# ModuRL/ModuRL_Gym

Measured on NVIDIA B200. Metric: env-steps/sec (CartPole-v1, 2^24 envs), higher is better.
Workload: dtype f32

## Files before the change

### modurl_gym_b200/csrc/mgym_api.cu

```cuda
#include <dlfcn.h>

#include <cmath>
#include <cstdarg>
#include <cstdio>
#include <cstdlib>
#include <cstring>
#include <limits>
#include <mutex>
#include <new>
#include <string>

#include "../../include/mgym.h"
#include "mgym_kernels.cuh"

#if defined(__has_include)
#if __has_include(<nccl.h>)
#include <nccl.h>
#define MGYM_HAVE_NCCL_H 1
#endif
#endif
namespace {
#ifdef MGYM_HAVE_NCCL_H
constexpr int kNcclFloat64 = (int)ncclFloat64, kNcclSum = (int)ncclSum;
static_assert(kNcclFloat64 == 8 && kNcclSum == 0, "NCCL enum values changed: update the header-less fallback below");
#else
constexpr int kNcclFloat64 = 8, kNcclSum = 0;
#endif
}

using namespace mgym;

struct mgym_env {
  int kind = 0;
  uint64_t n = 0;
  int device = 0;
  uint64_t seed = 0;
  mgym_config cfg{};
  int cnt_mode = CNT_U32;
  bool vec4 = false;

  float* state = nullptr;
  void* steps = nullptr;
  uint32_t* sbt = nullptr;
  float* ep_return = nullptr;
  float* reset_pool = nullptr;
  uint64_t pool_len = 0;
  unsigned long long* stats = nullptr;
  uint32_t* bad_action = nullptr;
  float* params = nullptr;
  bool redraw = false;
  float redraw_lo[MAX_PARAMS] = {}, redraw_hi[MAX_PARAMS] = {};

  uint64_t t = 0;
  uint64_t n_resets = 0;
  EnvConsts k{};
  int num_sms = 0;

  void* h_actions = nullptr;
  float* h_obs = nullptr;
  float* h_reward = nullptr;
  uint8_t* h_flags = nullptr;
  unsigned long long* work = nullptr;
  uint64_t work_issued[3] = {0, 0, 0};
  int work_slot = 0;
  unsigned long long* clock = nullptr;
  uint64_t call_tickets = 0;
  cudaStream_t pipe_stream[2] = {nullptr, nullptr};
  cudaEvent_t pipe_event[3] = {nullptr, nullptr, nullptr};
};

namespace {

thread_local std::string g_last_error;

int fail(int code, const char* fmt, ...) {
  char buf[512];
  va_list ap;
  va_start(ap, fmt);
  vsnprintf(buf, sizeof(buf), fmt, ap);
  va_end(ap);
  g_last_error = buf;
  return code;
}

#define MGYM_CUDA(expr)                                                                            \
  do {                                                                                             \
    cudaError_t e_ = (expr);                                                                       \
    if (e_ != cudaSuccess)                                                                         \
      return fail(e_ == cudaErrorMemoryAllocation ? MGYM_ERR_OUT_OF_MEMORY : MGYM_ERR_CUDA,        \
                  "%s failed: %s (%s:%d)", #expr, cudaGetErrorString(e_), __FILE__, __LINE__);    \
  } while (0)

struct DeviceGuard {
  int prev = -1;
  bool switched = false;
  explicit DeviceGuard(int dev) {
    if (cudaGetDevice(&prev) == cudaSuccess && prev != dev) switched = cudaSetDevice(dev) == cudaSuccess;
  }
  ~DeviceGuard() {
    if (switched) cudaSetDevice(prev);
  }
};

constexpr int kStateDim[MGYM_NUM_KINDS] = {4, 2, 2, 2, 4};
constexpr int kObsDim[MGYM_NUM_KINDS] = {4, 2, 2, 3, 6};
constexpr int kContinuous[MGYM_NUM_KINDS] = {0, 0, 1, 1, 0};
constexpr int kNumActions[MGYM_NUM_KINDS] = {2, 3, 0, 0, 3};
const char* const kNames[MGYM_NUM_KINDS] = {"CartPole-v1", "MountainCar-v0", "MountainCarContinuous-v0",
                                            "Pendulum-v1", "Acrobot-v1"};

constexpr int kNumParams[MGYM_NUM_KINDS] = {6, 2, 2, 3, 0};
const char* const kParamNames[MGYM_NUM_KINDS][6] = {
    {"gravity", "masscart", "masspole", "length", "force_mag", "tau"},
    {"force", "gravity"},
    {"power", "gravity"},
    {"g", "m", "l"},
    {}};
// ... 74 lines not shown
  p.n = e->n;
  p.first = 0;
  p.ld = e->n;
  p.seed = e->seed;
  p.keys = philox_keys(e->seed);
  p.t_dev = e->cfg.device_clock ? e->clock : nullptr;
  p.base_dev = nullptr;
  p.env_base = e->cfg.env_index_base;
  p.t = e->t;
  p.k = e->k;
  return p;
}

constexpr int kMaxDevices = 64;

struct OccupancyCache {
  static constexpr int kSlots = 256;
  std::mutex mu;
  const void* key[kSlots] = {};
  int dev[kSlots] = {};
  int per_sm[kSlots] = {};
  int used = 0;
  int find(const void* k, int d) {
    std::lock_guard<std::mutex> lock(mu);
    for (int i = 0; i < used; ++i)
      if (key[i] == k && dev[i] == d) return per_sm[i];
    return 0;
  }
  void put(const void* k, int d, int v) {
    std::lock_guard<std::mutex> lock(mu);
    if (used < kSlots) key[used] = k, dev[used] = d, per_sm[used] = v, ++used;
  }
};
OccupancyCache g_occupancy;

template <typename KP>
int launch_persistent(void (*kernel)(KP), const mgym_env* e, const KP& p, uint64_t groups, cudaStream_t st) {
  constexpr int threads = 256;
  int per_sm = g_occupancy.find(reinterpret_cast<const void*>(kernel), e->device);
  if (per_sm == 0) {
    MGYM_CUDA(cudaOccupancyMaxActiveBlocksPerMultiprocessor(&per_sm, kernel, threads, 0));
    if (per_sm < 1) per_sm = 1;
    g_occupancy.put(reinterpret_cast<const void*>(kernel), e->device, per_sm);
  }
  uint64_t blocks = (uint64_t)e->num_sms * per_sm;
  const uint64_t need = (groups + threads - 1) / threads;
  if (blocks > need) blocks = need;
  if (blocks < 1) blocks = 1;
  kernel<<<(unsigned)blocks, threads, 0, st>>>(p);
  MGYM_CUDA(cudaGetLastError());
  return MGYM_OK;
}

template <int KIND, int CNT, bool AUTO = true, bool PARAMS = false, bool REDRAW = false>
int launch_step_tma(const mgym_env* ce, const KParams<PARAMS, REDRAW>& p_in, cudaStream_t st) {
  mgym_env* e = const_cast<mgym_env*>(ce);
  KParams<PARAMS, REDRAW> p = p_in;
  using L = TmaLayout<KIND, CNT, AUTO, PARAMS>;
  auto kernel = step_kernel_tma<KIND, CNT, AUTO, PARAMS, REDRAW>;
  constexpr int threads = TMA_THREADS;
  static int cached_per_sm[kMaxDevices] = {};
  int per_sm = e->device < kMaxDevices ? cached_per_sm[e->device] : 0;
  if (per_sm == 0) {
    MGYM_CUDA(cudaFuncSetAttribute(kernel, cudaFuncAttributeMaxDynamicSharedMemorySize, (int)L::SMEM_BYTES));
    MGYM_CUDA(cudaOccupancyMaxActiveBlocksPerMultiprocessor(&per_sm, kernel, threads, L::SMEM_BYTES));
    if (per_sm < 1) per_sm = 1;
    if (e->device < kMaxDevices) cached_per_sm[e->device] = per_sm;
  }
  const uint64_t slots = (uint64_t)e->num_sms * per_sm;
  const uint64_t tiles = p.n / TMA_TILE;
  uint64_t blocks = tiles < slots ? tiles : slots;
  if (blocks < 1) blocks = 1;
  p.work_counter = e->work + e->work_slot;
  if (p.t_dev && e->work_slot == 0) {
    p.base_dev = e->clock + 1;
    if (p.adv_clock)
      p.adv_tickets = tiles + blocks;
    else
      e->call_tickets += tiles + blocks;
  } else {
    p.work_base = e->work_issued[e->work_slot];
    e->work_issued[e->work_slot] += tiles + blocks;
  }
  cudaLaunchConfig_t cfg{};
  cfg.gridDim = dim3((unsigned)blocks);
  cfg.blockDim = dim3(threads);
  cfg.dynamicSmemBytes = L::SMEM_BYTES;
  cfg.stream = st;
  cudaLaunchAttribute attr[1];
  attr[0].id = cudaLaunchAttributeProgrammaticStreamSerialization;
  attr[0].val.programmaticStreamSerializationAllowed = 1;
  cfg.attrs = attr;
  cfg.numAttrs = 1;
  MGYM_CUDA(cudaLaunchKernelEx(&cfg, kernel, p));
  return MGYM_OK;
}

template <int KIND, int V, bool ROLLOUT, bool PARAMS = false, bool REDRAW = false, bool FINAL = false>
int dispatch_mode(const mgym_env* e, const KParams<PARAMS, REDRAW>& p, cudaStream_t st) {
  static_assert(!FINAL || ROLLOUT, "final observations are a rollout form");
  const uint64_t groups = p.n / V;
  const bool autor = e->cfg.auto_reset != 0;
  if constexpr (!ROLLOUT && V == 4) {
    if constexpr (!REDRAW) {
      if (!autor && p.n % TMA_TILE == 0) return launch_step_tma<KIND, CNT_U32, false, PARAMS>(e, p, st);
    }
    if (autor && p.n % TMA_TILE == 0) {
      if constexpr (KIND == 0) {
        return launch_step_tma<KIND, CNT_S16, true, PARAMS, REDRAW>(e, p, st);
      } else {
        switch (e->cnt_mode) {
          case CNT_S16: return launch_step_tma<KIND, CNT_S16, true, PARAMS, REDRAW>(e, p, st);
          case CNT_S32_LAZY: return launch_step_tma<KIND, CNT_S32_LAZY, true, PARAMS, REDRAW>(e, p, st);
          default: return launch_step_tma<KIND, CNT_S32, true, PARAMS, REDRAW>(e, p, st);
        }
      }
    }
    if (p.n > TMA_TILE) {
      KParams<PARAMS, REDRAW> head = p, tail = p;
      head.adv_dt = 0;
      head.n = p.n - p.n % TMA_TILE;
      tail.first = p.first + head.n;
      tail.n = p.n - head.n;
      int rc = dispatch_mode<KIND, 4, false, PARAMS, REDRAW>(e, head, st);
      if (rc != MGYM_OK) return rc;
      return dispatch_mode<KIND, 4, false, PARAMS, REDRAW>(e, tail, st);
    }
  }
  [[maybe_unused]] const bool full = ROLLOUT && V == 4 && autor && p.n % (32 * V) == 0 && p.obs_out && p.reward_out &&
                                     p.flags_out;
#define MGYM_LAUNCH(AUTO_, CNT_)                                                                         \
  do {                                                                                                   \
    if constexpr (ROLLOUT) {                                                                             \
      if constexpr (AUTO_ && V == 4) {                                                                   \
        if (full)                                                                                        \
// ... 197 lines not shown
}

int mgym_space_action(int kind, float* low, float* high) {
  if (!valid_kind(kind) || !low || !high) return fail(MGYM_ERR_BAD_ARGUMENT, "mgym_space_action: bad argument");
  if (kind == MGYM_MOUNTAIN_CAR_CONTINUOUS_V0) {
    *low = -1.0f, *high = 1.0f;
  } else if (kind == MGYM_PENDULUM_V1) {
    *low = -2.0f, *high = 2.0f;
  } else {
    *low = 0.0f, *high = (float)(kNumActions[kind] - 1);
  }
  return MGYM_OK;
}

int mgym_config_default(int kind, mgym_config* cfg) {
  if (!valid_kind(kind) || !cfg) return fail(MGYM_ERR_BAD_ARGUMENT, "mgym_config_default: bad argument");
  memset(cfg, 0, sizeof(*cfg));
  cfg->struct_size = sizeof(mgym_config);
  cfg->auto_reset = 1;
  cfg->sutton_barto_reward = 0;
  cfg->is_euler = 1;
  cfg->goal_velocity = 0.0f;
  cfg->track_stats = 1;
  cfg->validate_actions = 0;
  cfg->env_index_base = 0;
  cfg->device_clock = 0;
  cfg->track_returns = 0;
  switch (kind) {
    case MGYM_MOUNTAIN_CAR_CONTINUOUS_V0: cfg->max_episode_steps = 999; break;
    case MGYM_PENDULUM_V1: cfg->max_episode_steps = 200; break;
    case MGYM_ACROBOT_V1: cfg->max_episode_steps = 500; break;
    default: cfg->max_episode_steps = 0;
  }
  return MGYM_OK;
}

int mgym_destroy(mgym_env* e) {
  if (!e) return MGYM_OK;
  DeviceGuard guard(e->device);
  cudaFree(e->clock);
  cudaFree(e->state);
  cudaFree(e->steps);
  cudaFree(e->sbt);
  cudaFree(e->ep_return);
  cudaFree(e->reset_pool);
  cudaFree(e->stats);
  cudaFree(e->bad_action);
  cudaFree(e->params);
  cudaFree(e->h_actions);
  cudaFree(e->h_obs);
  cudaFree(e->h_reward);
  cudaFree(e->h_flags);
  cudaFree(e->work);
  for (auto& s : e->pipe_stream)
    if (s) cudaStreamDestroy(s);
  for (auto& ev : e->pipe_event)
    if (ev) cudaEventDestroy(ev);
  delete e;
  return MGYM_OK;
}

int mgym_create(int kind, uint64_t num_envs, int device_ordinal, uint64_t seed, const mgym_config* cfg_in,
                mgym_env** out) {
  if (!out) return fail(MGYM_ERR_BAD_ARGUMENT, "mgym_create: out is NULL");
  *out = nullptr;
  if (!valid_kind(kind)) return fail(MGYM_ERR_BAD_ARGUMENT, "mgym_create: unknown kind %d", kind);
  if (num_envs == 0) return fail(MGYM_ERR_BAD_ARGUMENT, "mgym_create: num_envs must be > 0");
  mgym_config cfg;
  mgym_config_default(kind, &cfg);
  if (cfg_in) {
    if (cfg_in->struct_size != sizeof(mgym_config))
      return fail(MGYM_ERR_BAD_ARGUMENT, "mgym_create: cfg->struct_size %u != %zu", cfg_in->struct_size,
                  sizeof(mgym_config));
    cfg = *cfg_in;
  }
  if (cfg.max_episode_steps < 0) return fail(MGYM_ERR_BAD_ARGUMENT, "mgym_create: max_episode_steps < 0");

  int n_dev = 0;
  cudaError_t ce = cudaGetDeviceCount(&n_dev);
  if (ce != cudaSuccess || n_dev == 0)
    return fail(MGYM_ERR_CUDA, "mgym_create: no CUDA device (%s); there is no CPU fallback",
                ce == cudaSuccess ? "device count is 0" : cudaGetErrorString(ce));
  if (device_ordinal < 0 || device_ordinal >= n_dev)
    return fail(MGYM_ERR_BAD_ARGUMENT, "mgym_create: device %d out of range [0,%d)", device_ordinal, n_dev);

  mgym_env* e = new (std::nothrow) mgym_env();
  if (!e) return fail(MGYM_ERR_OUT_OF_MEMORY, "mgym_create: host allocation failed");
  e->kind = kind;
  e->n = num_envs;
  e->device = device_ordinal;
  e->seed = seed;
  e->cfg = cfg;
  e->k = make_consts(kind, cfg);
  e->vec4 = (num_envs % 4 == 0) && (cfg.env_index_base % 4 == 0);

  if (!cfg.auto_reset) {
    e->cnt_mode = CNT_U32;
  } else if (kind == MGYM_CARTPOLE_V1) {
    e->cnt_mode = CNT_S16;
  } else if (cfg.max_episode_steps > 0 && cfg.max_episode_steps <= 65535) {
    e->cnt_mode = CNT_S16;
  } else if (cfg.max_episode_steps > 65535) {
    e->cnt_mode = CNT_S32;
  } else {
    e->cnt_mode = CNT_S32_LAZY;
  }

  DeviceGuard guard(device_ordinal);
  int rc = [&]() -> int {
    cudaDeviceProp prop;
    MGYM_CUDA(cudaGetDeviceProperties(&prop, device_ordinal));
    e->num_sms = prop.multiProcessorCount;
    const size_t n = (size_t)num_envs;
    MGYM_CUDA(cudaMalloc(&e->state, sizeof(float) * kStateDim[kind] * n));
    MGYM_CUDA(cudaMemset(e->state, 0, sizeof(float) * kStateDim[kind] * n));
    MGYM_CUDA(cudaMalloc(&e->steps, counter_width(e->cnt_mode) * n));
    MGYM_CUDA(cudaMemset(e->steps, 0, counter_width(e->cnt_mode) * n));
    if (!cfg.auto_reset && kind == MGYM_CARTPOLE_V1) {
      MGYM_CUDA(cudaMalloc(&e->sbt, sizeof(uint32_t) * n));
      fill_u32_kernel<<<(unsigned)((n + 255) / 256), 256>>>(e->sbt, 1u, n);
      MGYM_CUDA(cudaGetLastError());
    }
    const bool analytic = kind == MGYM_CARTPOLE_V1 || kind == MGYM_MOUNTAIN_CAR_V0 || kind == MGYM_ACROBOT_V1;
    if (cfg.auto_reset && cfg.track_stats && cfg.track_returns && !analytic) {
      MGYM_CUDA(cudaMalloc(&e->ep_return, sizeof(float) * n));
      MGYM_CUDA(cudaMemset(e->ep_return, 0, sizeof(float) * n));
    }
    MGYM_CUDA(cudaMalloc(&e->stats, 5 * sizeof(unsigned long long)));
    MGYM_CUDA(cudaMemset(e->stats, 0, 5 * sizeof(unsigned long long)));
    MGYM_CUDA(cudaMalloc(&e->clock, 3 * sizeof(unsigned long long)));
    MGYM_CUDA(cudaMemset(e->clock, 0, 3 * sizeof(unsigned long long)));
    MGYM_CUDA(cudaMalloc(&e->work, 4 * sizeof(unsigned long long)));
    MGYM_CUDA(cudaMemset(e->work, 0, 4 * sizeof(unsigned long long)));
    MGYM_CUDA(cudaMalloc(&e->bad_action, sizeof(uint32_t)));
    MGYM_CUDA(cudaMemset(e->bad_action, 0, sizeof(uint32_t)));
    MGYM_CUDA(cudaDeviceSynchronize());
    return MGYM_OK;
  }();
  if (rc != MGYM_OK) {
    std::string keep = g_last_error;
    mgym_destroy(e);
    g_last_error = keep;
    return rc;
  }
  *out = e;
  return MGYM_OK;
}

uint64_t mgym_num_envs(const mgym_env* e) { return e ? e->n : 0; }
int mgym_kind_of(const mgym_env* e) { return e ? e->kind : MGYM_ERR_BAD_ARGUMENT; }
uint64_t mgym_step_index(const mgym_env* ce) {
  if (!ce) return 0;
  mgym_env* e = const_cast<mgym_env*>(ce);
  if (e->cfg.device_clock) {
    DeviceGuard guard(e->device);
    unsigned long long t = e->t;
    if (cudaDeviceSynchronize() == cudaSuccess &&
        cudaMemcpy(&t, e->clock, sizeof(t), cudaMemcpyDeviceToHost) == cudaSuccess)
      e->t = t;
    else
      cudaGetLastError();
  }
  return e->t;
}
float* mgym_state_ptr(mgym_env* e) { return e ? e->state : nullptr; }

int mgym_reset_masked(mgym_env* e, const uint8_t* mask, float* obs_out, void* stream) {
  if (e) {
    if (int rc = refuse_capture(e, (cudaStream_t)stream, "mgym_reset", false)) return rc;
  }
  if (!e) return fail(MGYM_ERR_BAD_ARGUMENT, "mgym_reset: env is NULL");
  DeviceGuard guard(e->device);
  cudaStream_t st = (cudaStream_t)stream;
  KernelParams p = base_params(e);
  p.obs_out = obs_out;
  int rc;
  switch (e->kind) {
    case 0: rc = launch_reset_kind<0>(e, p, mask, st); break;
    case 1: rc = launch_reset_kind<1>(e, p, mask, st); break;
    case 2: rc = launch_reset_kind<2>(e, p, mask, st); break;
    case 3: rc = launch_reset_kind<3>(e, p, mask, st); break;
    default: rc = launch_reset_kind<4>(e, p, mask, st); break;
  }
  if (rc == MGYM_OK && e->redraw) {
    reset_redraw_params_kernel<<<(unsigned)((e->n + 255) / 256), 256, 0, st>>>(
        e->params, e->n, kNumParams[e->kind], mask, e->seed, e->cfg.env_index_base, e->n_resets, redraw_box(e));
// ... 217 lines not shown
                (unsigned long long)h.pool_len, (unsigned long long)mine.pool_len);
  const bool with_params = (h.has_params & 1u) != 0 && kNumParams[e->kind] > 0;
  const bool with_ranges = with_params && (h.has_params & 2u) != 0;
  if (blob_bytes < checkpoint_bytes(e, with_params, with_ranges))
    return fail(MGYM_ERR_BAD_ARGUMENT, "mgym_checkpoint_load: truncated blob");
  float lo[MAX_PARAMS] = {}, hi[MAX_PARAMS] = {};
  if (with_ranges) {
    const size_t np = (size_t)kNumParams[e->kind];
    const uint8_t* r = static_cast<const uint8_t*>(blob) + checkpoint_bytes(e, true, false);
    memcpy(lo, r, sizeof(float) * np);
    memcpy(hi, r + sizeof(float) * np, sizeof(float) * np);
    if (int rc = check_redraw_ranges(e->kind, lo, hi, "mgym_checkpoint_load")) return rc;
  }
  DeviceGuard guard(e->device);
  if (with_params && !e->params) MGYM_CUDA(cudaMalloc(&e->params, param_bytes(e)));
  cudaStream_t st = (cudaStream_t)stream;
  const size_t n = (size_t)e->n;
  const uint8_t* in = static_cast<const uint8_t*>(blob) + sizeof(h);
  auto push = [&](void* dev, size_t bytes) -> int {
    if (bytes) MGYM_CUDA(cudaMemcpyAsync(dev, in, bytes, cudaMemcpyHostToDevice, st));
    in += bytes;
    return MGYM_OK;
  };
  int rc;
  if ((rc = push(e->state, sizeof(float) * kStateDim[e->kind] * n))) return rc;
  if ((rc = push(e->steps, counter_bytes(e)))) return rc;
  if ((rc = push(e->sbt, e->sbt ? sizeof(uint32_t) * n : 0))) return rc;
  if ((rc = push(e->ep_return, e->ep_return ? sizeof(float) * n : 0))) return rc;
  if ((rc = push(e->stats, 5 * sizeof(unsigned long long)))) return rc;
  if ((rc = push(e->params, with_params ? param_bytes(e) : 0))) return rc;
  MGYM_CUDA(cudaStreamSynchronize(st));
  if (!with_params) {
    cudaFree(e->params);
    e->params = nullptr;
  }
  e->redraw = with_ranges;
  memcpy(e->redraw_lo, lo, sizeof(lo));
  memcpy(e->redraw_hi, hi, sizeof(hi));
  e->seed = h.seed;
  e->t = h.t;
  if (e->cfg.device_clock) {
    const unsigned long long t = h.t;
    MGYM_CUDA(cudaMemcpyAsync(e->clock, &t, sizeof(t), cudaMemcpyHostToDevice, st));
    MGYM_CUDA(cudaStreamSynchronize(st));
  }
  e->n_resets = h.n_resets;
  return MGYM_OK;
}

int mgym_step(mgym_env* e, const void* actions, float* obs_out, float* reward_out, uint8_t* flags_out,
              float* final_obs_out, void* stream) {
  if (!e || !actions) return fail(MGYM_ERR_BAD_ARGUMENT, "mgym_step: NULL argument");
  e->work_slot = 0;
  DeviceGuard guard(e->device);
  cudaStream_t st = (cudaStream_t)stream;
  if (int rc = refuse_capture(e, st, "mgym_step", true)) return rc;
  if (int rc = validate_device_actions(e, actions, e->n, st)) return rc;
  e->call_tickets = 0;
  KernelParams p = base_params(e);
  p.actions = actions;
  p.obs_out = (obs_out == e->state) ? nullptr : obs_out;
  p.reward_out = reward_out;
  p.flags_out = flags_out;
  p.final_obs_out = final_obs_out;
  p.adv_clock = e->cfg.device_clock ? e->clock : nullptr;
  p.adv_dt = 1;
  const bool vec4 = e->vec4 && aligned16(actions) && aligned16(obs_out) && aligned16(reward_out) &&
                    aligned16(flags_out) && aligned16(final_obs_out);
  int rc = dispatch<false>(e, p, vec4, st);
  if (rc != MGYM_OK) return rc;
  return advance_clock(e, 1, st, true);
}

static int run_rollout(const char* fn, mgym_env* e, uint32_t K, const void* actions, float* obs_traj, float* reward_traj,
                       uint8_t* flags_traj, float* final_obs_traj, unsigned long long* done_count_out, void* stream) {
  if (!e) return fail(MGYM_ERR_BAD_ARGUMENT, "%s: env is NULL", fn);
  if (final_obs_traj) {
    if (!e->cfg.auto_reset)
      return fail(MGYM_ERR_BAD_ARGUMENT, "%s: a manual-mode handle resets nothing inside the rollout; obs_traj "
                  "already holds the final observations", fn);
    if (final_obs_traj == obs_traj)
      return fail(MGYM_ERR_BAD_ARGUMENT, "%s: final_obs_traj must not be obs_traj", fn);
  }
  if (K == 0) return MGYM_OK;
  DeviceGuard guard(e->device);
  cudaStream_t st = (cudaStream_t)stream;
  if (int rc = refuse_capture(e, st, fn, true)) return rc;
  if (int rc = validate_device_actions(e, actions, (uint64_t)K * e->n, st)) return rc;
  e->call_tickets = 0;
  KernelParams p = base_params(e);
  p.actions = actions;
  p.obs_out = obs_traj;
  p.reward_out = reward_traj;
  p.flags_out = flags_traj;
  p.done_count = done_count_out;
  p.K = K;
  p.adv_clock = e->cfg.device_clock ? e->clock : nullptr;
  p.adv_dt = K;
  if (done_count_out) MGYM_CUDA(cudaMemsetAsync(done_count_out, 0, sizeof(unsigned long long), st));
  const bool vec4 = e->vec4 && aligned16(actions) && aligned16(obs_traj) && aligned16(reward_traj) &&
                    aligned16(flags_traj);
  p.work_counter = e->work + 3;
  p.work_base = 0;
  MGYM_CUDA(cudaMemsetAsync(e->work + 3, 0, sizeof(unsigned long long), st));
  int rc;
  if (final_obs_traj) {
// ... 154 lines not shown
                  kParamNames[e->kind][c], (double)low[c], (double)high[c], pos ? ", low > 0" : "");
    box.lo[c] = (double)low[c];
    box.range[c] = (double)high[c] - (double)low[c];
  }
  if (!e->params && is_capturing(st))
    return fail(MGYM_ERR_BAD_ARGUMENT, "mgym_sample_params: set or sample the parameters once before capturing "
                "(the rows are allocated on first use)");
  if (int rc = ensure_params(e, st)) return rc;
  sample_params_kernel<<<(unsigned)((e->n + 255) / 256), 256, 0, st>>>(e->params, e->n, np, mask, e->seed,
                                                                       e->cfg.env_index_base, key, box);
  MGYM_CUDA(cudaGetLastError());
  return MGYM_OK;
}

int mgym_set_param_redraw(mgym_env* e, const float* low, const float* high, void* stream) {
  if (!e) return fail(MGYM_ERR_BAD_ARGUMENT, "mgym_set_param_redraw: env is NULL");
  if (kNumParams[e->kind] == 0) return no_params(e, "mgym_set_param_redraw");
  if (!low != !high)
    return fail(MGYM_ERR_BAD_ARGUMENT, "mgym_set_param_redraw: low and high must both be given, or both be NULL");
  DeviceGuard guard(e->device);
  cudaStream_t st = (cudaStream_t)stream;
  if (int rc = refuse_capture(e, st, "mgym_set_param_redraw", false)) return rc;
  if (!low) {
    e->redraw = false;
    return MGYM_OK;
  }
  if (int rc = check_redraw_ranges(e->kind, low, high, "mgym_set_param_redraw")) return rc;
  if (int rc = ensure_params(e, st)) return rc;
  for (int c = 0; c < MAX_PARAMS; ++c) {
    e->redraw_lo[c] = c < kNumParams[e->kind] ? low[c] : 0.0f;
    e->redraw_hi[c] = c < kNumParams[e->kind] ? high[c] : 0.0f;
  }
  e->redraw = true;
  return MGYM_OK;
}

int mgym_get_param_redraw(const mgym_env* e, int* enabled, float* low, float* high) {
  if (!e || !enabled) return fail(MGYM_ERR_BAD_ARGUMENT, "mgym_get_param_redraw: NULL argument");
  *enabled = e->redraw ? 1 : 0;
  for (int c = 0; e->redraw && c < kNumParams[e->kind]; ++c) {
    if (low) low[c] = e->redraw_lo[c];
    if (high) high[c] = e->redraw_hi[c];
  }
  return MGYM_OK;
}

int mgym_step_host(mgym_env* e, const void* actions_host, float* obs_host, float* reward_host, uint8_t* flags_host,
                   void* stream) {
  if (!e || !actions_host) return fail(MGYM_ERR_BAD_ARGUMENT, "mgym_step_host: NULL argument");
  DeviceGuard guard(e->device);
  cudaStream_t st = (cudaStream_t)stream;
  if (int rc = refuse_capture(e, st, "mgym_step_host", false)) return rc;
  e->call_tickets = 0;
  const size_t n = (size_t)e->n;
  if (e->cfg.validate_actions && !kContinuous[e->kind]) {
    const uint8_t* a = static_cast<const uint8_t*>(actions_host);
    const uint8_t lim = (uint8_t)kNumActions[e->kind];
    for (size_t i = 0; i < n; ++i)
      if (a[i] >= lim) return invalid_action(e);
  }
  const int od = kObsDim[e->kind];
  const size_t act = action_size(e->kind), asz = act * n, osz = sizeof(float) * od * n;
  const bool obs_is_state = kObsDim[e->kind] == kStateDim[e->kind];
  if (!e->h_actions) MGYM_CUDA(cudaMalloc(&e->h_actions, asz));
  if (obs_host && !obs_is_state && !e->h_obs) MGYM_CUDA(cudaMalloc(&e->h_obs, osz));
  if (reward_host && !e->h_reward) MGYM_CUDA(cudaMalloc(&e->h_reward, sizeof(float) * n));
  if (flags_host && !e->h_flags) MGYM_CUDA(cudaMalloc(&e->h_flags, n));
  float* dev_obs = obs_host ? (obs_is_state ? e->state : e->h_obs) : nullptr;

  constexpr size_t kMinChunk = 1u << 18;
  const size_t chunks = (n >= 2 * kMinChunk && e->vec4) ? (n / kMinChunk > 8 ? 8 : n / kMinChunk) : 1;
  if (chunks > 1 && !e->pipe_stream[0]) {
    for (auto& s : e->pipe_stream) MGYM_CUDA(cudaStreamCreateWithFlags(&s, cudaStreamNonBlocking));
    for (auto& ev : e->pipe_event) MGYM_CUDA(cudaEventCreateWithFlags(&ev, cudaEventDisableTiming));
  }
  if (chunks > 1) {
    MGYM_CUDA(cudaEventRecord(e->pipe_event[2], st));
    for (auto& s : e->pipe_stream) MGYM_CUDA(cudaStreamWaitEvent(s, e->pipe_event[2], 0));
  }
  const size_t per = ((n / chunks) / TMA_TILE) * TMA_TILE;
  for (size_t c = 0; c < chunks; ++c) {
    cudaStream_t cs = chunks > 1 ? e->pipe_stream[c & 1] : st;
    e->work_slot = chunks > 1 ? 1 + (int)(c & 1) : 0;
    const size_t b = c * per, cnt = (c + 1 == chunks) ? n - b : per;
    MGYM_CUDA(cudaMemcpyAsync((uint8_t*)e->h_actions + act * b, (const uint8_t*)actions_host + act * b, act * cnt,
                              cudaMemcpyHostToDevice, cs));
    KernelParams p = base_params(e);
    p.first = b;
    p.n = cnt;
    p.actions = e->h_actions;
    p.obs_out = (obs_host && !obs_is_state) ? e->h_obs : nullptr;
    p.reward_out = reward_host ? e->h_reward : nullptr;
    p.flags_out = flags_host ? e->h_flags : nullptr;
    int rc = dispatch<false>(e, p, e->vec4, cs);
    if (rc != MGYM_OK) return rc;
    if (obs_host)
      MGYM_CUDA(cudaMemcpy2DAsync(obs_host + b, sizeof(float) * n, dev_obs + b, sizeof(float) * n, sizeof(float) * cnt,
                                  (size_t)od, cudaMemcpyDeviceToHost, cs));
    if (reward_host)
      MGYM_CUDA(cudaMemcpyAsync(reward_host + b, e->h_reward + b, sizeof(float) * cnt, cudaMemcpyDeviceToHost, cs));
    if (flags_host) MGYM_CUDA(cudaMemcpyAsync(flags_host + b, e->h_flags + b, cnt, cudaMemcpyDeviceToHost, cs));
  }
  if (chunks > 1) {
    for (int i = 0; i < 2; ++i) {
      MGYM_CUDA(cudaEventRecord(e->pipe_event[i], e->pipe_stream[i]));
      MGYM_CUDA(cudaStreamWaitEvent(st, e->pipe_event[i], 0));
// ... 130 lines not shown
```

### modurl_gym_b200/csrc/mgym_kernels.cuh

```cuda
#pragma once

#include <type_traits>

#include "mgym_device.cuh"

namespace mgym {

template <int BYTES>
__device__ __forceinline__ void cp_async(uint32_t smem_dst, const void* gsrc) {
  static_assert(BYTES == 4 || BYTES == 16, "one lane's four actions");
  if constexpr (BYTES == 16) {
    asm volatile("cp.async.cg.shared.global [%0], [%1], 16;" ::"r"(smem_dst), "l"(gsrc) : "memory");
  } else {
    asm volatile("cp.async.ca.shared.global [%0], [%1], 4;" ::"r"(smem_dst), "l"(gsrc) : "memory");
  }
}
__device__ __forceinline__ void cp_async_commit() { asm volatile("cp.async.commit_group;" ::: "memory"); }
template <int PENDING>
__device__ __forceinline__ void cp_async_wait() {
  asm volatile("cp.async.wait_group %0;" ::"n"(PENDING) : "memory");
}

enum CounterMode : int { CNT_U32 = 2, CNT_S16 = 3, CNT_S32 = 4, CNT_S32_LAZY = 5 };
__host__ __device__ constexpr bool cnt_is_stamp(int c) { return c >= CNT_S16; }
__host__ __device__ constexpr bool cnt_is_lazy(int c) { return c == CNT_S32_LAZY; }
__host__ __device__ constexpr bool cnt_staged(int c) { return c != CNT_S32_LAZY; }

struct KernelParams {
  float* state;
  void* steps;
  uint32_t* sbt;
  float* ep_return;
  const void* actions;
  float* obs_out;
  float* reward_out;
  uint8_t* flags_out;
  float* final_obs_out;
  const float* reset_pool;
  uint64_t pool_len;
  unsigned long long* stats;
  unsigned long long* done_count;
  unsigned long long* work_counter;
  uint64_t work_base;
  const unsigned long long* t_dev;
  const unsigned long long* base_dev;
  unsigned long long* adv_clock;
  uint64_t adv_dt, adv_tickets;
  uint64_t n;
  uint64_t first;
  uint64_t ld;
  uint64_t seed, env_base, t;
  uint32_t K;
  PhiloxKeys keys;
  EnvConsts k;
};
struct KernelParamsP : KernelParams {
  const float* params;
};
constexpr int MAX_PARAMS = 8;
struct ParamBox {
  double lo[MAX_PARAMS], range[MAX_PARAMS];
};
struct KernelParamsR : KernelParamsP {
  ParamBox redraw;
};
template <bool PARAMS, bool REDRAW = false>
using KParams = std::conditional_t<REDRAW, KernelParamsR, std::conditional_t<PARAMS, KernelParamsP, KernelParams>>;

template <int NP>
__device__ __forceinline__ void redraw_params(const PhiloxKeys& ks, const ParamBox& box, uint64_t g, uint64_t t,
                                              uint32_t tag0, float* dst, uint64_t stride) {
#pragma unroll
  for (int b = 0; b * 4 < NP; ++b) {
    const uint4 w = philox_env(ks, g, t, tag0 + (uint32_t)b);
    const uint32_t ws[4] = {w.x, w.y, w.z, w.w};
#pragma unroll
    for (int j = 0; j < 4 && 4 * b + j < NP; ++j)
      dst[(uint64_t)(4 * b + j) * stride] = uniform_f64_to_f32(ws[j], box.lo[4 * b + j], box.range[4 * b + j]);
  }
}
struct RedrawDst {
  float* base;
  uint64_t cstride, vstride;
};

template <int NP_, int V>
struct ParamRows {
  static constexpr int NP = NP_;
  float r[NP_ > 0 ? NP_ : 1][V];
};
using NoParams = ParamRows<0, 1>;

__device__ __forceinline__ uint64_t launch_t(const KernelParams& p) { return p.t_dev ? *p.t_dev : p.t; }
__device__ __forceinline__ uint64_t launch_work_base(const KernelParams& p) {
  return p.base_dev ? *p.base_dev : p.work_base;
}
// ... 523 lines not shown
        Vec<float, V> o;
#pragma unroll
        for (int v = 0; v < V; ++v) o.v[v] = g.fin[v][c];
        stv<float, V>(p.final_obs_out + (uint64_t)c * p.ld + base, o);
      }
    }
    if (p.reward_out) {
      Vec<float, V> rw;
#pragma unroll
      for (int v = 0; v < V; ++v) rw.v[v] = g.reward[v];
      stv<float, V>(p.reward_out + base, rw);
    }
    if (p.flags_out) {
      Vec<uint8_t, V> fl;
#pragma unroll
      for (int v = 0; v < V; ++v) fl.v[v] = (uint8_t)g.flags[v];
      stv<uint8_t, V>(p.flags_out + base, fl);
    }
  }
  if constexpr (AUTO) stats_flush<KIND>(acc, p);
  fused_clock_advance(p);
}

namespace tma {
__device__ __forceinline__ uint32_t smem_u32(const void* p) { return (uint32_t)__cvta_generic_to_shared(p); }
__device__ __forceinline__ void mbar_init(uint32_t bar, uint32_t count) {
  asm volatile("mbarrier.init.shared::cta.b64 [%0], %1;" ::"r"(bar), "r"(count) : "memory");
}
__device__ __forceinline__ void fence_mbar_init() { asm volatile("fence.mbarrier_init.release.cluster;" ::: "memory"); }
__device__ __forceinline__ void mbar_expect_tx(uint32_t bar, uint32_t bytes) {
  asm volatile("mbarrier.arrive.expect_tx.shared::cta.b64 _, [%0], %1;" ::"r"(bar), "r"(bytes) : "memory");
}
__device__ __forceinline__ void bulk_g2s(uint32_t dst, const void* src, uint32_t bytes, uint32_t bar) {
  asm volatile("cp.async.bulk.shared::cluster.global.mbarrier::complete_tx::bytes [%0], [%1], %2, [%3];" ::"r"(dst),
               "l"(src), "r"(bytes), "r"(bar)
               : "memory");
}
__device__ __forceinline__ void mbar_arrive(uint32_t bar) {
  asm volatile("mbarrier.arrive.shared::cta.b64 _, [%0];" ::"r"(bar) : "memory");
}
__device__ __forceinline__ void mbar_wait(uint32_t bar, uint32_t parity) {
  asm volatile(
      "{\n"
      ".reg .pred P1;\n"
      "LAB_WAIT:\n"
      "mbarrier.try_wait.parity.shared::cta.b64 P1, [%0], %1;\n"
      "@P1 bra DONE;\n"
      "bra LAB_WAIT;\n"
      "DONE:\n"
      "}\n" ::"r"(bar),
      "r"(parity)
      : "memory");
}
}

constexpr int TMA_STAGES = 4;
constexpr int TMA_CONSUMER_WARPS = 8;
constexpr int TMA_THREADS = (TMA_CONSUMER_WARPS + 2) * 32;
constexpr int TMA_RESET_BUFFERS = 2;
constexpr int TMA_TILE = TMA_CONSUMER_WARPS * 32 * 4;

template <int KIND, int CNT, bool AUTO = true, bool PARAMS = false>
struct TmaLayout {
  using E = Env<KIND>;
  static constexpr uint32_t ROW = TMA_TILE * 4;
  static constexpr uint32_t OFF_ACT = E::SD * ROW;
  static constexpr uint32_t ACT_BYTES = TMA_TILE * sizeof(typename E::act_t);
  static constexpr uint32_t OFF_CNT = OFF_ACT + ACT_BYTES;
  static constexpr uint32_t CNT_BYTES = cnt_staged(CNT) ? TMA_TILE * sizeof(typename CounterType<CNT>::type) : 0;
  static constexpr uint32_t OFF_RET = OFF_CNT + CNT_BYTES;
  static constexpr uint32_t RET_BYTES = (E::ANALYTIC_RETURN || !AUTO) ? 0 : ROW;
  static constexpr uint32_t OFF_SBT = OFF_RET + RET_BYTES;
  static constexpr uint32_t SBT_BYTES = (!AUTO && KIND == 0) ? ROW : 0;
  static constexpr uint32_t OFF_PAR = OFF_SBT + SBT_BYTES;
  static constexpr uint32_t PAR_BYTES = PARAMS ? E::NP * ROW : 0;
  static constexpr uint32_t STAGE_BYTES = (OFF_PAR + PAR_BYTES + 127u) & ~127u;
  static constexpr uint32_t BAR_BYTES = 128;
  static_assert(24 * TMA_STAGES <= 128, "barriers and tile ids must fit BAR_BYTES");
  static constexpr uint32_t QUEUE_STRIDE = 32 + TMA_TILE * 2 + TMA_TILE * 4;
  static constexpr uint32_t QUEUE_BYTES = TMA_RESET_BUFFERS * QUEUE_STRIDE;
  static constexpr int fit_stages() {
    const uint32_t budget = 110u * 1024u - 256u - QUEUE_BYTES;
    const int s = (int)(budget / STAGE_BYTES);
    return s > TMA_STAGES ? TMA_STAGES : (s < 1 ? 1 : s);
  }
  static constexpr int STAGES = PARAMS ? fit_stages() : TMA_STAGES;
  static constexpr uint32_t OFF_QUEUE = BAR_BYTES + STAGES * STAGE_BYTES;
  static constexpr uint32_t SMEM_BYTES = 128 + OFF_QUEUE + QUEUE_BYTES;
};

template <int KIND, int CNT, bool AUTO = true, bool PARAMS = false, bool REDRAW = false>
__global__ void __launch_bounds__(TMA_THREADS, 2)
    step_kernel_tma(const __grid_constant__ KParams<PARAMS, REDRAW> p) {
  using E = Env<KIND>;
  using L = TmaLayout<KIND, CNT, AUTO, PARAMS>;
  using act_t = typename E::act_t;
  using cnt_t = typename CounterType<CNT>::type;
  constexpr int SD = E::SD, OD = E::OD, V = 4;
  constexpr int TMA_STAGES = L::STAGES;
  using PR = ParamRows<PARAMS ? E::NP : 0, V>;
  static_assert(!REDRAW || (PARAMS && AUTO), "redraw is a form of the auto-reset parameter kernels");
  static_assert(AUTO || !cnt_is_stamp(CNT), "manual mode keeps the reference's own counters");
  extern __shared__ uint8_t smem_raw[];
  const uint32_t smem_base = (tma::smem_u32(smem_raw) + 127u) & ~127u;
  const uint32_t warp = __shfl_sync(0xffffffffu, threadIdx.x >> 5, 0);
  const uint32_t lane = threadIdx.x & 31;
  const uint32_t full0 = smem_base, empty0 = smem_base + 8 * TMA_STAGES;
  volatile uint64_t* tile_slot =
      reinterpret_cast<volatile uint64_t*>(smem_raw + (smem_base + 16 * TMA_STAGES - tma::smem_u32(smem_raw)));
  constexpr uint32_t QSTRIDE = L::QUEUE_STRIDE;
  const uint32_t queue0 = smem_base + L::OFF_QUEUE;
  uint8_t* const queue_ptr = smem_raw + (queue0 - tma::smem_u32(smem_raw));
  auto q_tile = [&](uint32_t b) { return reinterpret_cast<volatile uint64_t*>(queue_ptr + b * QSTRIDE + 16); };
  auto q_count = [&](uint32_t b) { return reinterpret_cast<uint32_t*>(queue_ptr + b * QSTRIDE + 24); };
  auto q_items = [&](uint32_t b) { return reinterpret_cast<uint16_t*>(queue_ptr + b * QSTRIDE + 32); };
  auto q_lengths = [&](uint32_t b) { return reinterpret_cast<uint32_t*>(queue_ptr + b * QSTRIDE + 32 + TMA_TILE * 2); };
  const uint32_t data0 = smem_base + L::BAR_BYTES;
  const uint64_t n_tiles = p.n / TMA_TILE;
  const bool track_ret = AUTO && !E::ANALYTIC_RETURN && p.ep_return != nullptr;
  const bool want_final = p.final_obs_out != nullptr;
  constexpr bool HAS_SBT = !AUTO && KIND == 0;
  StatAcc acc;

  if (threadIdx.x == 0) {
#pragma unroll
    for (int s = 0; s < TMA_STAGES; ++s) {
      tma::mbar_init(full0 + 8 * s, 1);
      tma::mbar_init(empty0 + 8 * s, TMA_CONSUMER_WARPS);
    }
    for (int b = 0; b < TMA_RESET_BUFFERS; ++b) {
      tma::mbar_init(queue0 + b * QSTRIDE, TMA_CONSUMER_WARPS);
      tma::mbar_init(queue0 + b * QSTRIDE + 8, 1);
      *q_count(b) = 0u;
    }
    tma::fence_mbar_init();
  }
  __syncthreads();
  asm volatile("griddepcontrol.wait;" ::: "memory");
  asm volatile("griddepcontrol.launch_dependents;");
  const uint64_t t_now = launch_t(p), work_base = launch_work_base(p);

  if (warp == TMA_CONSUMER_WARPS) {
    if (lane == 0) {
      const act_t* actions = reinterpret_cast<const act_t*>(p.actions);
      const uint32_t tx =
          SD * L::ROW + L::ACT_BYTES + L::CNT_BYTES + (track_ret ? L::ROW : 0u) + L::SBT_BYTES + L::PAR_BYTES;
      for (uint32_t it = 0;; ++it) {
        const uint32_t s = it % TMA_STAGES, round = it / TMA_STAGES;
        tma::mbar_wait(empty0 + 8 * s, (round & 1u) ^ 1u);
        const uint64_t tile = atomicAdd(p.work_counter, 1ull) - work_base;
        const uint32_t bar = full0 + 8 * s, dst = data0 + s * L::STAGE_BYTES;
        tile_slot[s] = tile;
        if (tile >= n_tiles) {
          tma::mbar_arrive(bar);
          break;
        }
        const uint64_t e0 = p.first + tile * TMA_TILE;
        tma::mbar_expect_tx(bar, tx);
#pragma unroll
        for (int c = 0; c < SD; ++c) tma::bulk_g2s(dst + c * L::ROW, p.state + (uint64_t)c * p.ld + e0, L::ROW, bar);
        tma::bulk_g2s(dst + L::OFF_ACT, actions + e0, L::ACT_BYTES, bar);
        if constexpr (cnt_staged(CNT))
          tma::bulk_g2s(dst + L::OFF_CNT, reinterpret_cast<const cnt_t*>(p.steps) + e0, L::CNT_BYTES, bar);
        if constexpr (!E::ANALYTIC_RETURN && AUTO) {
          if (track_ret) tma::bulk_g2s(dst + L::OFF_RET, p.ep_return + e0, L::ROW, bar);
        }
        if constexpr (HAS_SBT) tma::bulk_g2s(dst + L::OFF_SBT, p.sbt + e0, L::ROW, bar);
        if constexpr (PARAMS) {
#pragma unroll
          for (int c = 0; c < E::NP; ++c)
            tma::bulk_g2s(dst + L::OFF_PAR + c * L::ROW, p.params + (uint64_t)c * p.ld + e0, L::ROW, bar);
        }
      }
    }
    __syncwarp();
  } else if (warp == TMA_CONSUMER_WARPS + 1) {
    for (uint32_t it = 0;; ++it) {
      const uint32_t qb = it % TMA_RESET_BUFFERS, qround = it / TMA_RESET_BUFFERS;
      const uint32_t q_full = queue0 + qb * QSTRIDE, q_empty = q_full + 8;
      tma::mbar_wait(q_full, qround & 1u);
      const uint64_t tile = *q_tile(qb);
      if (tile >= n_tiles) break;
      const uint32_t count = *q_count(qb);
      const uint16_t* items = q_items(qb);
      const uint32_t* lengths = q_lengths(qb);
      const uint64_t tile_base = p.first + tile * TMA_TILE;
      for (uint32_t j = lane; j < count; j += 32) {
        const uint64_t local = tile_base + items[j];
        const uint64_t gid = p.env_base + local;
        float ns[SD];
        if (p.reset_pool) {
          const uint64_t k = (gid + t_now) % p.pool_len;
#pragma unroll
          for (int c = 0; c < SD; ++c) ns[c] = p.reset_pool[(uint64_t)c * p.pool_len + k];
        } else {
          E::reset(philox_env(p.keys, gid, episode_start(t_now, lengths[j]), TAG_AUTO_RESET), ns);
        }
        if constexpr (REDRAW) {
          redraw_params<E::NP>(p.keys, p.redraw, gid, episode_start(t_now, lengths[j]), TAG_REDRAW_AUTO,
                               const_cast<float*>(p.params) + local, p.ld);
        }
#pragma unroll
        for (int c = 0; c < SD; ++c) p.state[(uint64_t)c * p.ld + local] = ns[c];
        if (p.obs_out) {
          float no[OD];
          E::obs(ns, no);
#pragma unroll
          for (int c = 0; c < OD; ++c) p.obs_out[(uint64_t)c * p.ld + local] = no[c];
        }
      }
      __syncwarp();
      if (lane == 0) {
        *q_count(qb) = 0u;
        tma::mbar_arrive(q_empty);
      }
    }
    __syncwarp();
  } else {
    const uint32_t tid = threadIdx.x;
    for (uint32_t it = 0;; ++it) {
      const uint32_t s = it % TMA_STAGES, parity = (it / TMA_STAGES) & 1u;
      tma::mbar_wait(full0 + 8 * s, parity);
      const uint64_t tile = tile_slot[s];
      const uint32_t qb = it % TMA_RESET_BUFFERS, qround = it / TMA_RESET_BUFFERS;
      const uint32_t q_full = queue0 + qb * QSTRIDE, q_empty = q_full + 8;
      tma::mbar_wait(q_empty, (qround & 1u) ^ 1u);
      if (tid == 0) *q_tile(qb) = tile;
      if (tile >= n_tiles) {
        __syncwarp();
        if (lane == 0) tma::mbar_arrive(q_full);
        break;
      }
      const uint64_t base = p.first + tile * TMA_TILE + tid * V;

      Group<KIND, V> g;
      act_t action[V];
      PR prm;
      {
        const uint8_t* st = smem_raw + (data0 + s * L::STAGE_BYTES - tma::smem_u32(smem_raw));
        if constexpr (PARAMS) {
#pragma unroll
          for (int c = 0; c < E::NP; ++c) {
            const Vec<float, V> r = ldv<float, V>(reinterpret_cast<const float*>(st + L::OFF_PAR + c * L::ROW) + tid * V);
#pragma unroll
            for (int v = 0; v < V; ++v) prm.r[c][v] = r.v[v];
          }
        }
        Vec<float, V> row[SD];
#pragma unroll
        for (int c = 0; c < SD; ++c) row[c] = ldv<float, V>(reinterpret_cast<const float*>(st + c * L::ROW) + tid * V);
        const Vec<act_t, V> a = ldv<act_t, V>(reinterpret_cast<const act_t*>(st + L::OFF_ACT) + tid * V);
        Vec<cnt_t, V> cnt;
        if constexpr (cnt_staged(CNT)) cnt = ldv<cnt_t, V>(reinterpret_cast<const cnt_t*>(st + L::OFF_CNT) + tid * V);
        Vec<float, V> er;
        if constexpr (!E::ANALYTIC_RETURN && AUTO) {
          if (track_ret) er = ldv<float, V>(reinterpret_cast<const float*>(st + L::OFF_RET) + tid * V);
        }
        Vec<uint32_t, V> sb;
        if constexpr (HAS_SBT) sb = ldv<uint32_t, V>(reinterpret_cast<const uint32_t*>(st + L::OFF_SBT) + tid * V);
#pragma unroll
        for (int v = 0; v < V; ++v) {
#pragma unroll
          for (int c = 0; c < SD; ++c) g.st[v][c] = row[c].v[v];
          action[v] = a.v[v];
          g.steps[v] = 0;
          g.sbt[v] = SBT_NONE;
          if constexpr (cnt_staged(CNT)) g.steps[v] = cnt_decode<CNT>(cnt.v[v], t_now);
          if constexpr (HAS_SBT) g.sbt[v] = sb.v[v];
          g.ret[v] = 0.0f;
// ... 46 lines not shown
        stv<float, V>(p.state + (uint64_t)c * p.ld + base, o);
      }
      if constexpr (!cnt_is_stamp(CNT)) {
        Vec<cnt_t, V> cnt;
#pragma unroll
        for (int v = 0; v < V; ++v) cnt.v[v] = (cnt_t)g.steps[v];
        stv<cnt_t, V>(reinterpret_cast<cnt_t*>(p.steps) + base, cnt);
      }
      if constexpr (!E::ANALYTIC_RETURN && AUTO) {
        if (track_ret) {
          Vec<float, V> er;
#pragma unroll
          for (int v = 0; v < V; ++v) er.v[v] = g.ret[v];
          stv<float, V>(p.ep_return + base, er);
        }
      }
      if constexpr (HAS_SBT) {
        Vec<uint32_t, V> sbo;
#pragma unroll
        for (int v = 0; v < V; ++v) sbo.v[v] = g.sbt[v];
        stv<uint32_t, V>(p.sbt + base, sbo);
      }
      if (p.obs_out) {
#pragma unroll
        for (int c = 0; c < OD; ++c) {
          Vec<float, V> o;
#pragma unroll
          for (int v = 0; v < V; ++v) o.v[v] = E::OBS_IS_STATE ? g.st[v][c < SD ? c : 0] : g.obs[v][c];
          stv<float, V>(p.obs_out + (uint64_t)c * p.ld + base, o);
        }
      }
      if (want_final) {
#pragma unroll
        for (int c = 0; c < OD; ++c) {
          Vec<float, V> o;
#pragma unroll
          for (int v = 0; v < V; ++v) o.v[v] = g.fin[v][c];
          stv<float, V>(p.final_obs_out + (uint64_t)c * p.ld + base, o);
        }
      }
      if (p.reward_out) {
        Vec<float, V> rw;
#pragma unroll
        for (int v = 0; v < V; ++v) rw.v[v] = g.reward[v];
        stv<float, V>(p.reward_out + base, rw);
      }
      if (p.flags_out) *reinterpret_cast<uint32_t*>(p.flags_out + base) = fw;
      __syncwarp();
      if (lane == 0) tma::mbar_arrive(q_full);
    }
  }
  if constexpr (AUTO) stats_flush<KIND>(acc, p);
  fused_clock_advance(p);
}

template <int KIND>
constexpr int rollout_min_blocks() {
  return KIND == 4 ? 2 : 3;
}

template <int KIND, int V, bool AUTO, int CNT, bool FULL, bool PARAMS = false, bool REDRAW = false, bool FINAL = false>
__global__ void __launch_bounds__(256, rollout_min_blocks<KIND>())
    rollout_kernel(const __grid_constant__ KParams<PARAMS, REDRAW> p) {
  using E = Env<KIND>;
  using act_t = typename E::act_t;
  using cnt_t = typename CounterType<CNT>::type;
  using PR = ParamRows<PARAMS ? E::NP : 0, V>;
  constexpr int SD = E::SD, OD = E::OD;
  static_assert(!REDRAW || (PARAMS && AUTO), "redraw is a form of the auto-reset parameter kernels");
  static_assert(!FULL || (AUTO && V == 4), "the FULL form is built for the vector auto-reset path only");
  static_assert(!FINAL || AUTO, "final observations exist only where the rollout resets");
  static_assert(!cnt_is_lazy(CNT) && (AUTO || !cnt_is_stamp(CNT)), "the host maps CNT_S32_LAZY to CNT_S32 here");
  constexpr int ACT_RING = PARAMS ? 4 : 8;
  __shared__ float par_slots[PARAMS ? E::NP * V : 1][PARAMS ? 256 : 1];
  static_assert((ACT_RING & (ACT_RING - 1)) == 0, "power of two");
  constexpr uint32_t RING_STRIDE = 256 * V * sizeof(act_t);
  __shared__ __align__(16) act_t act_ring[V == 4 ? ACT_RING : 1][256 * V];
  constexpr bool PREFETCH = AUTO && V == 4 && E::PREFETCH_RESETS;
  __shared__ float4 next_reset[PREFETCH ? 4 : 1][256];
  StatAcc acc;
  uint32_t dones = 0;
  const uint64_t groups = p.n / V;
  const bool track_ret = !E::ANALYTIC_RETURN && p.ep_return != nullptr;
  const bool policy = p.actions == nullptr;
  const act_t* actions = reinterpret_cast<const act_t*>(p.actions);
  const uint32_t lane = threadIdx.x & 31;
  const uint64_t t_first = launch_t(p);

  for (;;) {
    unsigned long long ticket = 0;
    if (lane == 0) ticket = atomicAdd(p.work_counter, 1ull) - p.work_base;
    ticket = __shfl_sync(0xffffffffu, ticket, 0);
    const uint64_t grp0 = ticket * 32;
    if (grp0 >= groups) break;
    const uint64_t grp = grp0 + lane;
    const bool active = FULL || grp < groups;
    const uint64_t base = p.first + (active ? grp * V : 0);
    Group<KIND, V> g;
#pragma unroll
    for (int v = 0; v < V; ++v) {
      g.steps[v] = 0;
      g.sbt[v] = SBT_NONE;
      g.ret[v] = 0.0f;
#pragma unroll
      for (int c = 0; c < SD; ++c) g.st[v][c] = 0.0f;
    }
// ... 635 lines not shown
```

Baseline: 152.3 billion.

## Overlap consecutive TMA step kernels via per-tile epoch flags instead of grid dependency wait

When the same env steps consecutively on the same stream, the next TMA step kernel skips the programmatic-dependent-launch grid wait. Instead its producer waits per tile on an epoch counter that the previous launch's reset warp publishes in batches once each tile is fully written. A global CTA-completion counter lets a launch fall back to the full grid wait once the previous launch is done or after a bounded spin. This aims to let consecutive steps' tiles overlap rather than serializing at kernel boundaries. In exchange it adds per-tile acquire loads, nanosleep spinning, alternating work-counter slots and a host-side mutex/map lookup per launch, with real memory-ordering risk across proxies.

After: 149.0 billion (median of 6 runs). 2.2% lower.

```diff
diff --git a/modurl_gym_b200/csrc/mgym_api.cu b/modurl_gym_b200/csrc/mgym_api.cu
--- a/modurl_gym_b200/csrc/mgym_api.cu
+++ b/modurl_gym_b200/csrc/mgym_api.cu
@@ -5,10 +5,14 @@
 #include <cstdio>
 #include <cstdlib>
 #include <cstring>
+#include <iterator>
 #include <limits>
+#include <map>
 #include <mutex>
 #include <new>
 #include <string>
+#include <thread>
+#include <tuple>
 
 #include "../../include/mgym.h"
 #include "mgym_kernels.cuh"
@@ -61,8 +65,12 @@
   float* h_reward = nullptr;
   uint8_t* h_flags = nullptr;
   unsigned long long* work = nullptr;
-  uint64_t work_issued[3] = {0, 0, 0};
+  uint64_t work_issued[5] = {0, 0, 0, 0, 0};
   int work_slot = 0;
+  uint32_t* tile_epoch = nullptr;
+  uint32_t seq = 0;
+  bool seq_taken = false;
+  uint64_t ctas_launched = 0;
   unsigned long long* clock = nullptr;
   uint64_t call_tickets = 0;
   cudaStream_t pipe_stream[2] = {nullptr, nullptr};
@@ -243,6 +251,28 @@
   return MGYM_OK;
 }
 
+class LastStepRecord {
+ public:
+  bool exchange(int device, cudaStream_t st, const mgym_env* e) {
+    const Key k{device, st, st == cudaStreamPerThread ? std::this_thread::get_id() : std::thread::id()};
+    std::lock_guard<std::mutex> lock(mu_);
+    const mgym_env*& last = last_[k];
+    const bool same = last == e;
+    last = e;
+    return same;
+  }
+  void forget(const mgym_env* e) {
+    std::lock_guard<std::mutex> lock(mu_);
+    for (auto it = last_.begin(); it != last_.end();) it = it->second == e ? last_.erase(it) : std::next(it);
+  }
+
+ private:
+  using Key = std::tuple<int, cudaStream_t, std::thread::id>;
+  std::mutex mu_;
+  std::map<Key, const mgym_env*> last_;
+};
+LastStepRecord g_last_step;
+
 template <int KIND, int CNT, bool AUTO = true, bool PARAMS = false, bool REDRAW = false>
 int launch_step_tma(const mgym_env* ce, const KParams<PARAMS, REDRAW>& p_in, cudaStream_t st) {
   mgym_env* e = const_cast<mgym_env*>(ce);
@@ -262,16 +292,31 @@
   const uint64_t tiles = p.n / TMA_TILE;
   uint64_t blocks = tiles < slots ? tiles : slots;
   if (blocks < 1) blocks = 1;
-  p.work_counter = e->work + e->work_slot;
-  if (p.t_dev && e->work_slot == 0) {
+  if (!e->seq_taken) {
+    e->seq += 1;
+    e->seq_taken = true;
+  }
+  p.tile_epoch = e->tile_epoch;
+  p.seq = e->seq;
+  p.early = 0;
+  p.ctas_done = e->work + 5;
+  p.ctas_before = e->ctas_launched;
+  e->ctas_launched += blocks;
+  const bool caller_stream = e->work_slot == 0;
+  const bool own_last = caller_stream && g_last_step.exchange(e->device, st, e);
+  if (p.t_dev && caller_stream) {
+    p.work_counter = e->work;
     p.base_dev = e->clock + 1;
     if (p.adv_clock)
       p.adv_tickets = tiles + blocks;
     else
       e->call_tickets += tiles + blocks;
   } else {
-    p.work_base = e->work_issued[e->work_slot];
-    e->work_issued[e->work_slot] += tiles + blocks;
+    const int slot = caller_stream ? ((e->seq & 1u) ? 4 : 0) : e->work_slot;
+    p.work_counter = e->work + slot;
+    p.work_base = e->work_issued[slot];
+    e->work_issued[slot] += tiles + blocks;
+    p.early = own_last ? 1u : 0u;
   }
   cudaLaunchConfig_t cfg{};
   cfg.gridDim = dim3((unsigned)blocks);
@@ -575,6 +620,8 @@
   cudaFree(e->h_reward);
   cudaFree(e->h_flags);
   cudaFree(e->work);
+  cudaFree(e->tile_epoch);
+  g_last_step.forget(e);
   for (auto& s : e->pipe_stream)
     if (s) cudaStreamDestroy(s);
   for (auto& ev : e->pipe_event)
@@ -653,8 +700,11 @@
     MGYM_CUDA(cudaMemset(e->stats, 0, 5 * sizeof(unsigned long long)));
     MGYM_CUDA(cudaMalloc(&e->clock, 3 * sizeof(unsigned long long)));
     MGYM_CUDA(cudaMemset(e->clock, 0, 3 * sizeof(unsigned long long)));
-    MGYM_CUDA(cudaMalloc(&e->work, 4 * sizeof(unsigned long long)));
-    MGYM_CUDA(cudaMemset(e->work, 0, 4 * sizeof(unsigned long long)));
+    MGYM_CUDA(cudaMalloc(&e->work, 6 * sizeof(unsigned long long)));
+    MGYM_CUDA(cudaMemset(e->work, 0, 6 * sizeof(unsigned long long)));
+    const size_t tiles = n / TMA_TILE + 1;
+    MGYM_CUDA(cudaMalloc(&e->tile_epoch, sizeof(uint32_t) * tiles));
+    MGYM_CUDA(cudaMemset(e->tile_epoch, 0, sizeof(uint32_t) * tiles));
     MGYM_CUDA(cudaMalloc(&e->bad_action, sizeof(uint32_t)));
     MGYM_CUDA(cudaMemset(e->bad_action, 0, sizeof(uint32_t)));
     MGYM_CUDA(cudaDeviceSynchronize());
@@ -978,6 +1028,7 @@
               float* final_obs_out, void* stream) {
   if (!e || !actions) return fail(MGYM_ERR_BAD_ARGUMENT, "mgym_step: NULL argument");
   e->work_slot = 0;
+  e->seq_taken = false;
   DeviceGuard guard(e->device);
   cudaStream_t st = (cudaStream_t)stream;
   if (int rc = refuse_capture(e, st, "mgym_step", true)) return rc;
@@ -1238,6 +1289,7 @@
   cudaStream_t st = (cudaStream_t)stream;
   if (int rc = refuse_capture(e, st, "mgym_step_host", false)) return rc;
   e->call_tickets = 0;
+  e->seq_taken = false;
   const size_t n = (size_t)e->n;
   if (e->cfg.validate_actions && !kContinuous[e->kind]) {
     const uint8_t* a = static_cast<const uint8_t*>(actions_host);
diff --git a/modurl_gym_b200/csrc/mgym_kernels.cuh b/modurl_gym_b200/csrc/mgym_kernels.cuh
--- a/modurl_gym_b200/csrc/mgym_kernels.cuh
+++ b/modurl_gym_b200/csrc/mgym_kernels.cuh
@@ -42,6 +42,11 @@
   unsigned long long* done_count;
   unsigned long long* work_counter;
   uint64_t work_base;
+  uint32_t* tile_epoch;
+  uint32_t seq;
+  uint32_t early;
+  unsigned long long* ctas_done;
+  uint64_t ctas_before;
   const unsigned long long* t_dev;
   const unsigned long long* base_dev;
   unsigned long long* adv_clock;
@@ -671,6 +676,44 @@
       "r"(parity)
       : "memory");
 }
+__device__ __forceinline__ uint32_t ld_acquire_gpu(const uint32_t* p) {
+  uint32_t v;
+  asm volatile("ld.acquire.gpu.global.u32 %0, [%1];" : "=r"(v) : "l"(p) : "memory");
+  return v;
+}
+__device__ __forceinline__ unsigned long long ld_acquire_gpu(const unsigned long long* p) {
+  unsigned long long v;
+  asm volatile("ld.acquire.gpu.global.u64 %0, [%1];" : "=l"(v) : "l"(p) : "memory");
+  return v;
+}
+__device__ __forceinline__ void red_release_gpu_add(unsigned long long* p, unsigned long long v) {
+  asm volatile("red.release.gpu.global.add.u64 [%0], %1;" ::"l"(p), "l"(v) : "memory");
+}
+__device__ __forceinline__ unsigned long long ld_relaxed_gpu(const unsigned long long* p) {
+  unsigned long long v;
+  asm volatile("ld.relaxed.gpu.global.u64 %0, [%1];" : "=l"(v) : "l"(p) : "memory");
+  return v;
+}
+__device__ __forceinline__ void st_relaxed_gpu(uint32_t* p, uint32_t v) {
+  asm volatile("st.relaxed.gpu.global.u32 [%0], %1;" ::"l"(p), "r"(v) : "memory");
+}
+__device__ __forceinline__ void fence_acq_rel_gpu() { asm volatile("fence.acq_rel.gpu;" ::: "memory"); }
+__device__ __forceinline__ void fence_proxy_async_global() { asm volatile("fence.proxy.async.global;" ::: "memory"); }
+__device__ __forceinline__ void grid_dependency_wait() { asm volatile("griddepcontrol.wait;" ::: "memory"); }
+}
+
+constexpr uint32_t OVERLAP_SPINS = 1u << 13;
+template <typename Cond>
+__device__ __forceinline__ void wait_or_settle(bool& settled, Cond cond) {
+  if (settled) return;
+  for (uint32_t i = 0; !cond(); ++i) {
+    if (i == OVERLAP_SPINS) {
+      tma::grid_dependency_wait();
+      settled = true;
+      return;
+    }
+    __nanosleep(128);
+  }
 }
 
 constexpr int TMA_STAGES = 4;
@@ -755,7 +798,7 @@
     tma::fence_mbar_init();
   }
   __syncthreads();
-  asm volatile("griddepcontrol.wait;" ::: "memory");
+  if (!p.early) tma::grid_dependency_wait();
   asm volatile("griddepcontrol.launch_dependents;");
   const uint64_t t_now = launch_t(p), work_base = launch_work_base(p);
 
@@ -764,6 +807,13 @@
       const act_t* actions = reinterpret_cast<const act_t*>(p.actions);
       const uint32_t tx =
           SD * L::ROW + L::ACT_BYTES + L::CNT_BYTES + (track_ret ? L::ROW : 0u) + L::SBT_BYTES + L::PAR_BYTES;
+      const uint32_t* epoch = p.tile_epoch + p.first / TMA_TILE;
+      bool settled = !p.early;
+      if (!settled) {
+        settled = tma::ld_acquire_gpu(p.ctas_done) >= p.ctas_before;
+        if (settled) tma::fence_proxy_async_global();
+      }
+      wait_or_settle(settled, [&] { return tma::ld_relaxed_gpu(p.work_counter) >= work_base; });
       for (uint32_t it = 0;; ++it) {
         const uint32_t s = it % TMA_STAGES, round = it / TMA_STAGES;
         tma::mbar_wait(empty0 + 8 * s, (round & 1u) ^ 1u);
@@ -775,6 +825,11 @@
           break;
         }
         const uint64_t e0 = p.first + tile * TMA_TILE;
+        if (!settled) {
+          settled = tma::ld_acquire_gpu(p.ctas_done) >= p.ctas_before;
+          wait_or_settle(settled, [&] { return (int32_t)(tma::ld_acquire_gpu(epoch + tile) - (p.seq - 1u)) >= 0; });
+          tma::fence_proxy_async_global();
+        }
         tma::mbar_expect_tx(bar, tx);
 #pragma unroll
         for (int c = 0; c < SD; ++c) tma::bulk_g2s(dst + c * L::ROW, p.state + (uint64_t)c * p.ld + e0, L::ROW, bar);
@@ -794,6 +849,15 @@
     }
     __syncwarp();
   } else if (warp == TMA_CONSUMER_WARPS + 1) {
+    constexpr uint32_t EPOCH_BATCH = 8;
+    uint32_t* const epoch = p.tile_epoch + p.first / TMA_TILE;
+    uint32_t pending[EPOCH_BATCH];
+    uint32_t n_pending = 0;
+    auto publish = [&] {
+      tma::fence_acq_rel_gpu();
+      for (uint32_t k = 0; k < n_pending; ++k) tma::st_relaxed_gpu(epoch + pending[k], p.seq);
+      n_pending = 0;
+    };
     for (uint32_t it = 0;; ++it) {
       const uint32_t qb = it % TMA_RESET_BUFFERS, qround = it / TMA_RESET_BUFFERS;
       const uint32_t q_full = queue0 + qb * QSTRIDE, q_empty = q_full + 8;
@@ -832,8 +896,11 @@
       if (lane == 0) {
         *q_count(qb) = 0u;
         tma::mbar_arrive(q_empty);
-      }
-    }
+        pending[n_pending++] = (uint32_t)tile;
+        if (n_pending == EPOCH_BATCH) publish();
+      }
+    }
+    if (lane == 0 && n_pending) publish();
     __syncwarp();
   } else {
     const uint32_t tid = threadIdx.x;
@@ -986,6 +1053,9 @@
   }
   if constexpr (AUTO) stats_flush<KIND>(acc, p);
   fused_clock_advance(p);
+  if (p.early) tma::grid_dependency_wait();
+  __syncthreads();
+  if (threadIdx.x == 0) tma::red_release_gpu_add(p.ctas_done, 1ull);
 }
 
 template <int KIND>
```
